# jakobblaabjerg/point-cloud-classifier

Measured on NVIDIA B200. Metric: train samples/sec (fwd+bwd), DeepSets B=256 N=1024, higher is better.
Workload: dtype bf16

## Files before the change

### point-cloud-classifier_b200/csrc/pcc_fused_bwd.cu

```cuda
#include "pcc_fused.cuh"
#include "pcc_head.cuh"

namespace pcc {

constexpr int kRingB = 3;

struct BwdParams {
  const float* x;
  const int64_t* offsets;
  int64_t n, B, num_tiles;
  int d, L, pooling, res_mask;
  const uint8_t* wpack;
  uint32_t w_off[kMaxLayers], wt_off[kMaxLayers];
  const float* bias[kMaxLayers];
  const float* dpooled;
  const int32_t* argmax;
  uint8_t* stage_h[kMaxLayers];
  uint8_t* stage_g[kMaxLayers];
  float* part_w[kMaxLayers];
  float* part_b[kMaxLayers];
  int virt;
  int nbig;
  const int32_t* row_set;
  const float* row_scale;
  long long* trace;
};

__device__ __forceinline__ void trace_b(long long* trace, int role, int& n, int id) {
  if (trace && blockIdx.x == 0 && n < 2047) {
    trace[role * 4096 + 2 * n] = id;
    trace[role * 4096 + 2 * n + 1] = clock64();
    ++n;
  }
}

struct BwdSmem {
  uint32_t bufG, bufH, ring, bias, bars, total;
};
__host__ __device__ inline BwdSmem bwd_smem(int H, int L) {
  BwdSmem s;
  uint32_t o = 0;
  s.bufG = o; o += kTileM * H * 2;
  s.bufH = o; o += kTileM * H * 2;
  s.ring = o; o += kRingB * w_slab_bytes(H);
  s.bias = o; o += (uint32_t)(L - 1) * H * 4;
  s.bars = o; o += 128;
  s.total = o;
  return s;
}

template <int H, int ACT>
__global__ void __launch_bounds__(kThreads, 1) phi_bwd_chain_kernel(const BwdParams p) {
  extern __shared__ __align__(1024) uint8_t smem[];
  const BwdSmem lay = bwd_smem(H, p.L);
  uint8_t* bufG = smem + lay.bufG;
  uint8_t* bufH = smem + lay.bufH;
  uint8_t* ring = smem + lay.ring;
  float* biasS = reinterpret_cast<float*>(smem + lay.bias);
  uint64_t* bars = reinterpret_cast<uint64_t*>(smem + lay.bars);
  uint64_t* full = bars;
  uint64_t* empty = bars + kRingB;
  uint64_t* a_ready = bars + 2 * kRingB;
  uint64_t* accA_ready = bars + 2 * kRingB + 1;
  uint64_t* accB_ready = bars + 2 * kRingB + 2;
  uint64_t* wf_ready = bars + 2 * kRingB + 3;
  uint32_t* tmem_slot = reinterpret_cast<uint32_t*>(bars + 2 * kRingB + 4);

  constexpr uint32_t SLAB = w_slab_bytes(H);
  constexpr uint32_t X_LBO = kTileM * 16;
  constexpr uint32_t W0_LBO = H * 16;
  constexpr uint32_t BLOB = kTileM * H * 2;
  constexpr int NSLAB = H / 64;
  constexpr int NCHUNK = H / 32;
  constexpr uint32_t ACC_A = 0, ACC_B = 256;

  const int warp = threadIdx.x >> 5, lane = threadIdx.x & 31;
  const int L = p.L;
  const int lh = L - 2;

  for (int i = threadIdx.x; i < (L - 1) * H; i += kThreads) biasS[i] = __ldg(p.bias[i / H] + (i % H));
  if (threadIdx.x == 0) {
    for (int i = 0; i < kRingB; ++i) { mbar_init(&full[i], 1); mbar_init(&empty[i], 1); }
    mbar_init(a_ready, kEpiWarps);
    mbar_init(accA_ready, 1);
    mbar_init(accB_ready, 1);
    mbar_init(wf_ready, 1);
    fence_mbar_init();
  }
  if (warp == kMmaWarp) tmem_alloc<512>(tmem_slot);
  tc_fence_before();
  __syncthreads();
  tc_fence_after();
  const uint32_t tmem = *tmem_slot;
  pdl_wait();
  const bool virt = p.virt != 0;
  const bool vmax = p.virt == 1, bcast = p.virt == 2;
  const bool bcast3 = bcast && p.L == 3;

  if (warp == kProdWarp) {
    if (lane == 0) {
      uint32_t stage = 0, phase = 0;
      auto push = [&](const uint8_t* src, uint32_t bytes) {
        mbar_wait(&empty[stage], phase ^ 1);
        mbar_arrive_expect_tx(&full[stage], bytes);
        bulk_g2s(ring + stage * SLAB, src, bytes, &full[stage]);
        if (++stage == kRingB) { stage = 0; phase ^= 1; }
      };
      auto push_layer = [&](uint32_t off) { for (int s = 0; s < NSLAB; ++s) push(p.wpack + off + (size_t)s * SLAB, SLAB); };
      for (int64_t tile = blockIdx.x; tile < p.num_tiles; tile += gridDim.x) {
        push(p.wpack + p.w_off[0], (kK0 / 8) * W0_LBO);
        if (!virt) push_layer(p.wt_off[L - 1]);
        if (L == 3) {
          push_layer(p.w_off[1]);
          push_layer(p.wt_off[1]);
          if (!bcast3) push(p.wpack + p.w_off[0], (kK0 / 8) * W0_LBO);
        }
      }
    }
  } else if (warp == kMmaWarp) {
    if (lane == 0) {
      constexpr uint32_t IDESC = make_idesc_bf16(128, H, 0, 0);
      uint32_t stage = 0, phase = 0, a_phase = 0;
      const uint32_t g_base = smem_u32(bufG), h_base = smem_u32(bufH), r_base = smem_u32(ring);
      auto wait_a = [&]() { mbar_wait(a_ready, a_phase); a_phase ^= 1; tc_fence_after(); };
      auto gemm = [&](uint32_t act_base, uint32_t acc_col, bool accumulate_first) {
        for (int s = 0; s < NSLAB; ++s) {
          mbar_wait(&full[stage], phase);
          tc_fence_after();
          const uint32_t w_slab = r_base + stage * SLAB;
#pragma unroll
          for (int ks = 0; ks < 4; ++ks)
            umma_bf16(tmem + acc_col, make_smem_desc_sw128_k(act_base + s * kActSlab + ks * 32),
                      make_smem_desc_sw128_k(w_slab + ks * 32), IDESC, ((s | ks) != 0) || accumulate_first);
          umma_commit(&empty[stage]);
          if (++stage == kRingB) { stage = 0; phase ^= 1; }
        }
      };
      auto gemm0 = [&]() {
        mbar_wait(&full[stage], phase);
        tc_fence_after();
        umma_bf16(tmem + ACC_A, make_smem_desc(h_base, X_LBO, 128), make_smem_desc(r_base + stage * SLAB, W0_LBO, 128),
                  IDESC, 0);
        umma_commit(&empty[stage]);
        if (++stage == kRingB) { stage = 0; phase ^= 1; }
      };
      for (int64_t tile = blockIdx.x; tile < p.num_tiles; tile += gridDim.x) {
        wait_a();
        gemm0();
        umma_commit(accA_ready);
        if (!virt) {
          wait_a();
          gemm(g_base, ACC_B, false);
          umma_commit(accB_ready);
        }
        if (L == 3) {
          wait_a();
          gemm(h_base, ACC_A, false);
          umma_commit(accA_ready);
          wait_a();
          gemm(bcast3 ? h_base : g_base, ACC_B, (p.res_mask >> 1) & 1);
          umma_commit(accB_ready);
          if (!bcast3) {
            wait_a();
            gemm0();
            umma_commit(accA_ready);
          }
        }
      }
    }
  } else {
    const int quarter = warp & 3, grp = warp >> 2;
    const int r = quarter * 32 + lane;
    const uint32_t lane_base = tmem + ((uint32_t)(quarter * 32) << 16);
    uint32_t phA = 0, phB = 0, wf_phase = 0;
    const int d = p.d;
    float xcur[kK0] = {}, xnext[kK0];
    auto load_x = [&](int64_t tile) {
      const int64_t row = tile * kTileM + r;
#pragma unroll
      for (int j = 0; j < kK0; ++j)
        xnext[j] = (grp == 0 && j < d && row < p.n && tile < p.num_tiles) ? __ldg(p.x + row * d + j) : 0.f;
    };
    auto stage_x = [&]() {
      if (grp == 0) {
        *reinterpret_cast<uint4*>(bufH + r * 16) = make_uint4(pack_bf16x2(xcur[0], xcur[1]), pack_bf16x2(xcur[2], xcur[3]),
                                                              pack_bf16x2(xcur[4], xcur[5]), pack_bf16x2(xcur[6], xcur[7]));
        *reinterpret_cast<uint4*>(bufH + X_LBO + r * 16) =
            make_uint4(pack_bf16x2(xcur[8], xcur[9]), pack_bf16x2(xcur[10], xcur[11]), pack_bf16x2(xcur[12], xcur[13]),
                       pack_bf16x2(xcur[14], xcur[15]));
      }
    };
    auto acquire = [&]() {
      if (threadIdx.x == 0) bulk_wait_read0();
      asm volatile("bar.sync 1, 256;" ::: "memory");
    };
    auto store_blob = [&](uint8_t* gdst, const uint8_t* sbuf) {
      fence_proxy_async();
      asm volatile("bar.sync 1, 256;" ::: "memory");
      if (threadIdx.x == 0) { bulk_s2g(gdst, sbuf, BLOB); bulk_commit(); }
    };
    auto store_slabs = [&](uint8_t* gdst, const uint8_t* sbuf, int s0, int count, uint8_t* gdst2, const uint8_t* sbuf2) {
      fence_proxy_async();
      asm volatile("bar.sync 1, 256;" ::: "memory");
      if (threadIdx.x == 0) {
        bulk_s2g(gdst + (size_t)s0 * kActSlab, sbuf + (size_t)s0 * kActSlab, (uint32_t)count * kActSlab);
        if (gdst2) bulk_s2g(gdst2 + (size_t)s0 * kActSlab, sbuf2 + (size_t)s0 * kActSlab, (uint32_t)count * kActSlab);
        bulk_commit();
      }
    };
    auto wait_A = [&]() { mbar_wait(accA_ready, phA); phA ^= 1; tc_fence_after(); };
    auto wait_B = [&]() { mbar_wait(accB_ready, phB); phB ^= 1; tc_fence_after(); };
    auto arrive_a = [&]() { tc_fence_before(); fence_proxy_async(); mbar_arrive_warp(a_ready); };
    auto h_chunk8 = [&](const uint32_t* z, const float* bl, uint8_t* dst, bool res) {
      const float4 b0 = *reinterpret_cast<const float4*>(bl);
      const float4 b1 = *reinterpret_cast<const float4*>(bl + 4);
      const uint64_t bb[4] = {f32x2(b0.x, b0.y), f32x2(b0.z, b0.w), f32x2(b1.x, b1.y), f32x2(b1.z, b1.w)};
      uint4 old = make_uint4(0u, 0u, 0u, 0u);
      if (res) old = *reinterpret_cast<const uint4*>(dst);
      const uint32_t oo[4] = {old.x, old.y, old.z, old.w};
      uint32_t pk[4];
#pragma unroll
      for (int j = 0; j < 4; ++j) {
        uint64_t o = act2<ACT>(fadd2(f32x2(__uint_as_float(z[2 * j]), __uint_as_float(z[2 * j + 1])), bb[j]));
        if (res) o = fadd2(o, bf16x2_to_f32x2(oo[j]));
        pk[j] = pack_bf16x2_pair(o);
      }
      *reinterpret_cast<uint4*>(dst) = make_uint4(pk[0], pk[1], pk[2], pk[3]);
    };
    auto hda_chunk8 = [&](const uint32_t* z, const float* bl, uint8_t* hdst, uint8_t* dadst) {
      const float4 b0 = *reinterpret_cast<const float4*>(bl);
      const float4 b1 = *reinterpret_cast<const float4*>(bl + 4);
      const uint64_t bb[4] = {f32x2(b0.x, b0.y), f32x2(b0.z, b0.w), f32x2(b1.x, b1.y), f32x2(b1.z, b1.w)};
      uint32_t ph[4], pd[4];
#pragma unroll
      for (int j = 0; j < 4; ++j) {
        uint64_t a, da;
        act_and_grad2<ACT>(fadd2(f32x2(__uint_as_float(z[2 * j]), __uint_as_float(z[2 * j + 1])), bb[j]), a, da);
        ph[j] = pack_bf16x2_pair(a);
        pd[j] = pack_bf16x2_pair(da);
      }
      *reinterpret_cast<uint4*>(hdst) = make_uint4(ph[0], ph[1], ph[2], ph[3]);
      *reinterpret_cast<uint4*>(dadst) = make_uint4(pd[0], pd[1], pd[2], pd[3]);
    };
    auto dz_chunk8 = [&](const uint32_t* z, const uint32_t* g, const float* bl, uint8_t* dst) {
      const float4 b0 = *reinterpret_cast<const float4*>(bl);
      const float4 b1 = *reinterpret_cast<const float4*>(bl + 4);
      const uint64_t bb[4] = {f32x2(b0.x, b0.y), f32x2(b0.z, b0.w), f32x2(b1.x, b1.y), f32x2(b1.z, b1.w)};
      uint32_t pk[4];
#pragma unroll
      for (int j = 0; j < 4; ++j) {
        uint64_t a, da;
        act_and_grad2<ACT>(fadd2(f32x2(__uint_as_float(z[2 * j]), __uint_as_float(z[2 * j + 1])), bb[j]), a, da);
        pk[j] = pack_bf16x2_pair(fmul2(f32x2(__uint_as_float(g[2 * j]), __uint_as_float(g[2 * j + 1])), da));
      }
      *reinterpret_cast<uint4*>(dst) = make_uint4(pk[0], pk[1], pk[2], pk[3]);
    };
    auto hdz_chunk8 = [&](const uint32_t* z, const uint32_t* g, const float* bl, uint8_t* hdst, uint8_t* gdst, bool res) {
      const float4 b0 = *reinterpret_cast<const float4*>(bl);
      const float4 b1 = *reinterpret_cast<const float4*>(bl + 4);
      const uint64_t bb[4] = {f32x2(b0.x, b0.y), f32x2(b0.z, b0.w), f32x2(b1.x, b1.y), f32x2(b1.z, b1.w)};
      uint4 old = make_uint4(0u, 0u, 0u, 0u);
      if (res) old = *reinterpret_cast<const uint4*>(hdst);
      const uint32_t oo[4] = {old.x, old.y, old.z, old.w};
      uint32_t ph[4], pg[4];
#pragma unroll
      for (int j = 0; j < 4; ++j) {
        uint64_t a, da;
        act_and_grad2<ACT>(fadd2(f32x2(__uint_as_float(z[2 * j]), __uint_as_float(z[2 * j + 1])), bb[j]), a, da);
        if (res) a = fadd2(a, bf16x2_to_f32x2(oo[j]));
        ph[j] = pack_bf16x2_pair(a);
        pg[j] = pack_bf16x2_pair(fmul2(f32x2(__uint_as_float(g[2 * j]), __uint_as_float(g[2 * j + 1])), da));
      }
      *reinterpret_cast<uint4*>(hdst) = make_uint4(ph[0], ph[1], ph[2], ph[3]);
      *reinterpret_cast<uint4*>(gdst) = make_uint4(pg[0], pg[1], pg[2], pg[3]);
    };

    load_x(blockIdx.x);
    int tn = 0;
    const bool tr0 = threadIdx.x == 0;
#define TRE(id) do { if (tr0) trace_b(p.trace, 0, tn, id); } while (0)
    for (int64_t tile = blockIdx.x; tile < p.num_tiles; tile += gridDim.x) {
      const int64_t r0 = tile * kTileM;
      const int64_t row = r0 + r;
#pragma unroll
      for (int j = 0; j < kK0; ++j) xcur[j] = xnext[j];
      TRE(0);
      stage_x();
      arrive_a();
      TRE(2);
      load_x(tile + gridDim.x);
      const int64_t myset = (!vmax && row < p.n) ? (int64_t)__ldg(p.row_set + row) : -1;
      const float scale = (!vmax && row < p.n) ? __ldg(p.row_scale + row) : 0.f;
      const float gs = vmax ? ((row < p.n) ? __ldg(p.dpooled + row) : 0.f) : 1.f;

      acquire();
      TRE(1);
      if (vmax) {
        if (threadIdx.x == 0) {
          const uint32_t f0 = (uint32_t)(r0 % H);
          mbar_arrive_expect_tx(wf_ready, NSLAB * kActSlab);
          for (int s = 0; s < NSLAB; ++s)
            bulk_g2s(bufG + s * kActSlab, p.wpack + p.w_off[L - 1] + (size_t)s * SLAB + (size_t)f0 * 128, kActSlab, wf_ready);
        }
      } else if (!bcast3) {
        float* gS = reinterpret_cast<float*>(bufH + 16384);
        int* aS = reinterpret_cast<int*>(bufH + 16384 + H * 4);
        const int64_t last_row = (r0 + kTileM - 1 < p.n - 1) ? r0 + kTileM - 1 : p.n - 1;
        const int64_t b_lo = __ldg(p.row_set + r0), b_hi = __ldg(p.row_set + last_row);
        const bool is_max = (p.pooling == PCC_POOL_MAX) && !bcast;
        if (myset < 0) {
          for (int kc = grp; kc < H / 8; kc += 2)
            *reinterpret_cast<uint4*>(bufG + act_chunk_off(r, kc * 8)) = make_uint4(0u, 0u, 0u, 0u);
        }
        for (int64_t b = (b_lo < 0 ? 0 : b_lo); b <= b_hi; ++b) {
          asm volatile("bar.sync 1, 256;" ::: "memory");
          for (int i = threadIdx.x; i < H; i += kEpiThreads) {
            gS[i] = __ldg(p.dpooled + b * H + i);
            if (is_max) aS[i] = __ldg(p.argmax + b * H + i);
          }
          asm volatile("bar.sync 1, 256;" ::: "memory");
          if (myset == b) {
            const int rr = (int)row;
#pragma unroll 2
            for (int kc = grp; kc < H / 8; kc += 2) {
              const float4 g0 = *reinterpret_cast<const float4*>(gS + kc * 8);
              const float4 g1 = *reinterpret_cast<const float4*>(gS + kc * 8 + 4);
              float o[8] = {g0.x, g0.y, g0.z, g0.w, g1.x, g1.y, g1.z, g1.w};
              if (is_max) {
                const int4 a0 = *reinterpret_cast<const int4*>(aS + kc * 8);
                const int4 a1 = *reinterpret_cast<const int4*>(aS + kc * 8 + 4);
                o[0] = a0.x == rr ? o[0] : 0.f; o[1] = a0.y == rr ? o[1] : 0.f; o[2] = a0.z == rr ? o[2] : 0.f;
                o[3] = a0.w == rr ? o[3] : 0.f; o[4] = a1.x == rr ? o[4] : 0.f; o[5] = a1.y == rr ? o[5] : 0.f;
                o[6] = a1.z == rr ? o[6] : 0.f; o[7] = a1.w == rr ? o[7] : 0.f;
              } else {
#pragma unroll
                for (int j = 0; j < 8; ++j) o[j] *= scale;
              }
              *reinterpret_cast<uint4*>(bufG + act_chunk_off(r, kc * 8)) =
                  make_uint4(pack_bf16x2(o[0], o[1]), pack_bf16x2(o[2], o[3]), pack_bf16x2(o[4], o[5]), pack_bf16x2(o[6], o[7]));
            }
          }
        }
      }
      TRE(3);
      if (!virt) {
        store_blob(p.stage_g[L - 1] + (size_t)tile * BLOB, bufG);
        arrive_a();
      }
      TRE(4);

      if (bcast3) {
        wait_A();
        TRE(5);
        const float* bl = biasS;
#pragma unroll 1
        for (int c = grp; c < NCHUNK; c += 2) {
          uint32_t z[32];
          tmem_ld32(lane_base + ACC_A + c * 32, z);
          tmem_wait_ld();
#pragma unroll
          for (int q = 0; q < 4; ++q) {
            const uint32_t off = act_chunk_off(r, c * 32 + q * 8);
            hda_chunk8(z + q * 8, bl + c * 32 + q * 8, bufH + off, bufG + off);
          }
          store_slabs(p.stage_h[0] + (size_t)tile * BLOB, bufH, c >> 1, 1, nullptr, nullptr);
        }
        TRE(6);
        arrive_a();
        TRE(7);
      } else if (L == 3) {
        wait_A();
        TRE(5);
        const float* bl = biasS;
        uint32_t va[32], vb[32];
        tmem_ld32(lane_base + ACC_A + grp * 32, va);
#pragma unroll 1
        for (int c = grp; c < NCHUNK; c += 4) {
          tmem_wait_ld();
          if (c + 2 < NCHUNK) tmem_ld32(lane_base + ACC_A + (c + 2) * 32, vb);
#pragma unroll
          for (int q = 0; q < 4; ++q) h_chunk8(va + q * 8, bl + c * 32 + q * 8, bufH + act_chunk_off(r, c * 32 + q * 8), false);
          if (c + 2 < NCHUNK) {
            tmem_wait_ld();
            if (c + 4 < NCHUNK) tmem_ld32(lane_base + ACC_A + (c + 4) * 32, va);
#pragma unroll
            for (int q = 0; q < 4; ++q)
              h_chunk8(vb + q * 8, bl + (c + 2) * 32 + q * 8, bufH + act_chunk_off(r, (c + 2) * 32 + q * 8), false);
          }
          store_slabs(p.stage_h[0] + (size_t)tile * BLOB, bufH, (c - grp) >> 1, (c + 2 < NCHUNK) ? 2 : 1, nullptr, nullptr);
        }
        TRE(6);
        arrive_a();
        TRE(7);
      }

      if (!virt) wait_B();
      TRE(8);
      wait_A();
      TRE(9);
      acquire();
      TRE(10);
      if (bcast3) {
        const bool res = (p.res_mask >> lh) & 1;
        const float* bl = biasS + lh * H;
        const float* grow = p.dpooled + (myset < 0 ? 0 : myset) * H;
        const float sc = myset < 0 ? 0.f : scale;
        uint32_t gn[32];
        auto load_g = [&](int c, uint32_t (&dst)[32]) {
#pragma unroll
          for (int j = 0; j < 8; ++j) {
            const float4 t4 = __ldg(reinterpret_cast<const float4*>(grow + c * 32) + j);
            dst[4 * j] = __float_as_uint(t4.x); dst[4 * j + 1] = __float_as_uint(t4.y);
            dst[4 * j + 2] = __float_as_uint(t4.z); dst[4 * j + 3] = __float_as_uint(t4.w);
          }
        };
        load_g(grp, gn);
#pragma unroll 1
        for (int c = grp; c < NCHUNK; c += 2) {
          uint32_t z[32], g[32];
          tmem_ld32(lane_base + ACC_A + c * 32, z);
#pragma unroll
          for (int j = 0; j < 32; ++j) g[j] = __float_as_uint(sc * __uint_as_float(gn[j]));
          if (c + 2 < NCHUNK) load_g(c + 2, gn);
          if (res) tmem_st32(lane_base + ACC_B + c * 32, g);
          tmem_wait_ld();
#pragma unroll
          for (int q = 0; q < 4; ++q)
            dz_chunk8(z + q * 8, g + q * 8, bl + c * 32 + q * 8, bufH + act_chunk_off(r, c * 32 + q * 8));
          store_slabs(p.stage_g[lh] + (size_t)tile * BLOB, bufH, c >> 1, 1, nullptr, nullptr);
        }
        if (res) tmem_wait_st();
      } else if (virt) {
        if (vmax) {
          mbar_wait(wf_ready, wf_phase);
          wf_phase ^= 1;
        }
        const bool res = (p.res_mask >> lh) & 1;
        const float* bl = biasS + lh * H;
#pragma unroll 1
        for (int c = grp; c < NCHUNK; c += 2) {
          uint32_t z[32], g[32];
          tmem_ld32(lane_base + ACC_A + c * 32, z);
#pragma unroll
          for (int q = 0; q < 4; ++q) {
            const uint4 wv = *reinterpret_cast<const uint4*>(bufG + act_chunk_off(r, c * 32 + q * 8));
            g[q * 8 + 0] = __float_as_uint(gs * bf16_lo(wv.x)); g[q * 8 + 1] = __float_as_uint(gs * bf16_hi(wv.x));
            g[q * 8 + 2] = __float_as_uint(gs * bf16_lo(wv.y)); g[q * 8 + 3] = __float_as_uint(gs * bf16_hi(wv.y));
            g[q * 8 + 4] = __float_as_uint(gs * bf16_lo(wv.z)); g[q * 8 + 5] = __float_as_uint(gs * bf16_hi(wv.z));
            g[q * 8 + 6] = __float_as_uint(gs * bf16_lo(wv.w)); g[q * 8 + 7] = __float_as_uint(gs * bf16_hi(wv.w));
          }
          if (res) tmem_st32(lane_base + ACC_B + c * 32, g);
          tmem_wait_ld();
#pragma unroll
          for (int q = 0; q < 4; ++q) {
            const uint32_t off = act_chunk_off(r, c * 32 + q * 8);
            if (bcast) dz_chunk8(z + q * 8, g + q * 8, bl + c * 32 + q * 8, bufG + off);
            else hdz_chunk8(z + q * 8, g + q * 8, bl + c * 32 + q * 8, bufH + off, bufG + off, res);
          }
          if (bcast) store_slabs(p.stage_g[lh] + (size_t)tile * BLOB, bufG, c >> 1, 1, nullptr, nullptr);
          else store_slabs(p.stage_h[lh] + (size_t)tile * BLOB, bufH, c >> 1, 1, p.stage_g[lh] + (size_t)tile * BLOB, bufG);
        }
        if (res) tmem_wait_st();
      } else {
        const bool res = (p.res_mask >> lh) & 1;
        const float* bl = biasS + lh * H;
#pragma unroll 1
        for (int c = grp; c < NCHUNK; c += 2) {
          uint32_t z[32], g[32];
          tmem_ld32(lane_base + ACC_A + c * 32, z);
          tmem_ld32(lane_base + ACC_B + c * 32, g);
          tmem_wait_ld();
#pragma unroll
          for (int q = 0; q < 4; ++q) {
            const uint32_t off = act_chunk_off(r, c * 32 + q * 8);
            hdz_chunk8(z + q * 8, g + q * 8, bl + c * 32 + q * 8, bufH + off, bufG + off, res);
          }
          store_slabs(p.stage_h[lh] + (size_t)tile * BLOB, bufH, c >> 1, 1, p.stage_g[lh] + (size_t)tile * BLOB, bufG);
        }
      }
      TRE(11);
      TRE(12);

      if (L == 3) {
        arrive_a();
        if (threadIdx.x == 0) bulk_wait_read0();
        asm volatile("bar.sync 1, 256;" ::: "memory");
        TRE(13);
        if (bcast3) {
          wait_B();
          TRE(14);
          TRE(15);
#pragma unroll 1
          for (int c = grp; c < NCHUNK; c += 2) {
            uint32_t g[32];
            tmem_ld32(lane_base + ACC_B + c * 32, g);
            tmem_wait_ld();
#pragma unroll
            for (int q = 0; q < 4; ++q) {
              uint8_t* dst = bufG + act_chunk_off(r, c * 32 + q * 8);
              const uint4 da = *reinterpret_cast<const uint4*>(dst);
              const uint32_t dd[4] = {da.x, da.y, da.z, da.w};
              uint32_t pk[4];
#pragma unroll
              for (int j = 0; j < 4; ++j)
                pk[j] = pack_bf16x2_pair(fmul2(f32x2(__uint_as_float(g[q * 8 + 2 * j]), __uint_as_float(g[q * 8 + 2 * j + 1])),
                                               bf16x2_to_f32x2(dd[j])));
              *reinterpret_cast<uint4*>(dst) = make_uint4(pk[0], pk[1], pk[2], pk[3]);
            }
            store_slabs(p.stage_g[0] + (size_t)tile * BLOB, bufG, c >> 1, 1, nullptr, nullptr);
          }
        } else {
        stage_x();
        arrive_a();
        wait_B();
        wait_A();
        TRE(14);
        acquire();
        TRE(15);
        const float* bl = biasS;
#pragma unroll 1
        for (int c = grp; c < NCHUNK; c += 2) {
          uint32_t z[32], g[32];
          tmem_ld32(lane_base + ACC_A + c * 32, z);
          tmem_ld32(lane_base + ACC_B + c * 32, g);
          tmem_wait_ld();
#pragma unroll
          for (int q = 0; q < 4; ++q)
            dz_chunk8(z + q * 8, g + q * 8, bl + c * 32 + q * 8, bufG + act_chunk_off(r, c * 32 + q * 8));
          store_slabs(p.stage_g[0] + (size_t)tile * BLOB, bufG, c >> 1, 1, nullptr, nullptr);
        }
        }
        TRE(16);
        TRE(17);
      }
    }
#undef TRE
    if (threadIdx.x == 0) bulk_wait0();
  }

  tc_fence_before();
  __syncthreads();
  if (warp == kMmaWarp) tmem_dealloc<512>(tmem);
}

constexpr int kSlots = 6;

struct WgradJob {
  int layer;
  int64_t first, stride;
  int slot;
};
__host__ __device__ inline int wgrad_members(int grid, int nbig, int layer) {
  if (layer == 0) return grid;
  return (grid - (layer - 1) + nbig - 1) / nbig;
}
__device__ inline WgradJob wgrad_job(int j, int cta, int grid, int nbig) {
  WgradJob w;
  if (j == 0) {
    w.layer = 1 + cta % nbig;
    w.first = cta / nbig;
    w.stride = wgrad_members(grid, nbig, w.layer);
    w.slot = cta / nbig;
  } else {
    w.layer = 0; w.first = cta; w.stride = grid; w.slot = cta;
  }
  return w;
}

__device__ __forceinline__ int64_t wgrad_last_tile(const WgradJob& jb, int64_t num_tiles) {
  if (jb.first >= num_tiles) return jb.first - jb.stride;
  return jb.first + (num_tiles - 1 - jb.first) / jb.stride * jb.stride;
}

template <int H>
__global__ void __launch_bounds__(kThreads, 1) phi_wgrad_kernel(const BwdParams p) {
  extern __shared__ __align__(1024) uint8_t smem[];
  constexpr uint32_t BLOB = kTileM * H * 2;
  constexpr uint32_t HBLOB = BLOB / 2;
  constexpr uint32_t HSLAB = kActSlab / 2;
  constexpr int NSL = H / 64;
  constexpr uint32_t XBLOB = kTileM * kK0 * 2;
  constexpr int HALVES = H / 128;
  constexpr int CH = H / 8;
  constexpr int CPW = CH / kEpiWarps;
  uint8_t* slots = smem;
  uint8_t* bufX = smem + kSlots * HBLOB;
  uint64_t* bars = reinterpret_cast<uint64_t*>(smem + kSlots * HBLOB + 2 * XBLOB);
  uint64_t* full = bars;
  uint64_t* empty = bars + kSlots;
  uint64_t* x_full = bars + 2 * kSlots;
  uint64_t* x_empty = bars + 2 * kSlots + 2;
  uint64_t* acc_ready = bars + 2 * kSlots + 4;
  uint64_t* acc_free = bars + 2 * kSlots + 5;
  uint32_t* tmem_slot = reinterpret_cast<uint32_t*>(bars + 2 * kSlots + 6);

  const int warp = threadIdx.x >> 5, lane = threadIdx.x & 31;
  const int j0 = (p.nbig == 0) ? 1 : 0;
  if (threadIdx.x == 0) {
    for (int i = 0; i < kSlots; ++i) { mbar_init(&full[i], 1); mbar_init(&empty[i], 1 + kEpiWarps); }
    for (int i = 0; i < 2; ++i) { mbar_init(&x_full[i], kEpiWarps); mbar_init(&x_empty[i], 1); }
    mbar_init(acc_ready, 1);
    mbar_init(acc_free, kEpiWarps);
    fence_mbar_init();
  }
  if (warp == kMmaWarp) tmem_alloc<512>(tmem_slot);
  tc_fence_before();
  __syncthreads();
  tc_fence_after();
  const uint32_t tmem = *tmem_slot;
  pdl_wait();

  if (warp == kProdWarp) {
    if (lane == 0) {
      uint32_t stage = 0, phase = 0;
      auto push = [&](const uint8_t* src, int hf) {
        mbar_wait(&empty[stage], phase ^ 1);
        mbar_arrive_expect_tx(&full[stage], HBLOB);
        for (int sl = 0; sl < NSL; ++sl)
          bulk_g2s(slots + stage * HBLOB + sl * HSLAB, src + (size_t)sl * kActSlab + (size_t)hf * HSLAB, HSLAB, &full[stage]);
        if (++stage == kSlots) { stage = 0; phase ^= 1; }
      };
      for (int j = 1; j >= j0; --j) {
        const WgradJob jb = wgrad_job(j, blockIdx.x, gridDim.x, p.nbig);
        const int l = jb.layer;
        for (int64_t tile = wgrad_last_tile(jb, p.num_tiles); tile >= jb.first; tile -= jb.stride) {
          for (int hf = 0; hf < 2; ++hf) {
            push(p.stage_g[l] + (size_t)tile * BLOB, hf);
            if (l >= 1) push(p.stage_h[l - 1] + (size_t)tile * BLOB, hf);
          }
        }
      }
    }
  } else if (warp == kMmaWarp) {
    if (lane == 0) {
      uint32_t stage = 0, phase = 0, xpar = 0, xphase = 0 , free_phase = 0;
      const uint32_t s_base = smem_u32(slots), x_base = smem_u32(bufX);
      for (int j = 1; j >= j0; --j) {
        const WgradJob jb = wgrad_job(j, blockIdx.x, gridDim.x, p.nbig);
        const int l = jb.layer;
        const int Np = (l == 0) ? kK0 : H;
        const uint32_t idesc = make_idesc_bf16(128, Np, 1, 1);
        if (j < 1) { mbar_wait(acc_free, free_phase); free_phase ^= 1; tc_fence_after(); }
        bool first = true;
        for (int64_t tile = wgrad_last_tile(jb, p.num_tiles); tile >= jb.first; tile -= jb.stride) {
          uint32_t x_addr = 0;
          if (l == 0) {
            mbar_wait(&x_full[xpar], (xphase >> xpar) & 1);
            xphase ^= 1u << xpar;
            x_addr = x_base + xpar * XBLOB;
          }
          for (int hf = 0; hf < 2; ++hf) {
            const uint32_t g_stage = stage;
            mbar_wait(&full[stage], phase);
            if (++stage == kSlots) { stage = 0; phase ^= 1; }
            uint32_t in_addr = 0, in_stage = 0;
            if (l >= 1) {
              in_stage = stage;
              mbar_wait(&full[stage], phase);
              if (++stage == kSlots) { stage = 0; phase ^= 1; }
              in_addr = s_base + in_stage * HBLOB;
            }
            tc_fence_after();
            const uint32_t g_addr = s_base + g_stage * HBLOB;
#pragma unroll
            for (int o = 0; o < HALVES; ++o)
              for (int ks = 0; ks < kTileM / 32; ++ks) {
                const uint64_t a_desc = make_smem_desc_sw128_mn(g_addr + o * (2 * HSLAB) + ks * 2048, HSLAB);
                const uint64_t b_desc = (l >= 1) ? make_smem_desc_sw128_mn(in_addr + ks * 2048, HSLAB)
                                                 : make_smem_desc(x_addr + (hf * (kTileM / 32) + ks) * 256, 128, kTileM * 16);
                umma_bf16(tmem + o * Np, a_desc, b_desc, idesc, !(first && hf == 0 && ks == 0));
              }
            umma_commit(&empty[g_stage]);
            if (l >= 1) umma_commit(&empty[in_stage]);
          }
          first = false;
          if (l == 0) { umma_commit(&x_empty[xpar]); xpar ^= 1; }
        }
        umma_commit(acc_ready);
      }
    }
  } else {
    const int quarter = warp & 3, grp = warp >> 2;
    const int r = quarter * 32 + lane;
    const uint32_t lane_base = tmem + ((uint32_t)(quarter * 32) << 16);
    uint32_t stage = 0, phase = 0, xpar = 0, xphase = 0, acc_phase = 0;
    const int d = p.d;
    for (int j = 1; j >= j0; --j) {
      const WgradJob jb = wgrad_job(j, blockIdx.x, gridDim.x, p.nbig);
      const int l = jb.layer;
      const int Np = (l == 0) ? kK0 : H;
      float dbacc[CPW][8];
#pragma unroll
      for (int i = 0; i < CPW; ++i)
#pragma unroll
        for (int j = 0; j < 8; ++j) dbacc[i][j] = 0.f;
      for (int64_t tile = wgrad_last_tile(jb, p.num_tiles); tile >= jb.first; tile -= jb.stride) {
        if (l == 0) {
          mbar_wait(&x_empty[xpar], ((xphase >> xpar) & 1) ^ 1);
          xphase ^= 1u << xpar;
          if (grp == 0) {
            const int64_t row = tile * kTileM + r;
            float xr[kK0];
#pragma unroll
            for (int j = 0; j < kK0; ++j) xr[j] = (j < d && row < p.n) ? __ldg(p.x + row * d + j) : 0.f;
            uint8_t* xb = bufX + xpar * XBLOB;
            *reinterpret_cast<uint4*>(xb + r * 16) = make_uint4(pack_bf16x2(xr[0], xr[1]), pack_bf16x2(xr[2], xr[3]),
                                                                pack_bf16x2(xr[4], xr[5]), pack_bf16x2(xr[6], xr[7]));
            *reinterpret_cast<uint4*>(xb + kTileM * 16 + r * 16) =
                make_uint4(pack_bf16x2(xr[8], xr[9]), pack_bf16x2(xr[10], xr[11]), pack_bf16x2(xr[12], xr[13]),
                           pack_bf16x2(xr[14], xr[15]));
          }
          fence_proxy_async();
          mbar_arrive_warp(&x_full[xpar]);
          xpar ^= 1;
        }
        for (int hf = 0; hf < 2; ++hf) {
          mbar_wait(&full[stage], phase);
          const uint8_t* gb = slots + stage * HBLOB;
#pragma unroll
          for (int i = 0; i < CPW; ++i) {
            const int c = warp + kEpiWarps * i;
#pragma unroll
            for (int rr = 0; rr < 2; ++rr) {
              const int rw = lane + 32 * rr;
              const uint4 u = *reinterpret_cast<const uint4*>(gb + (uint32_t)(c >> 3) * HSLAB + (uint32_t)rw * 128u +
                                                              ((uint32_t)((c & 7) ^ (rw & 7)) << 4));
              dbacc[i][0] += bf16_lo(u.x); dbacc[i][1] += bf16_hi(u.x); dbacc[i][2] += bf16_lo(u.y); dbacc[i][3] += bf16_hi(u.y);
              dbacc[i][4] += bf16_lo(u.z); dbacc[i][5] += bf16_hi(u.z); dbacc[i][6] += bf16_lo(u.w); dbacc[i][7] += bf16_hi(u.w);
            }
          }
          mbar_arrive_warp(&empty[stage]);
          if (++stage == kSlots) { stage = 0; phase ^= 1; }
          if (l >= 1) {
            mbar_wait(&full[stage], phase);
            mbar_arrive_warp(&empty[stage]);
            if (++stage == kSlots) { stage = 0; phase ^= 1; }
          }
        }
      }
      float* pb = p.part_b[l] + (size_t)jb.slot * H;
#pragma unroll
      for (int i = 0; i < CPW; ++i)
#pragma unroll
        for (int j = 0; j < 8; ++j) {
          float s = warp_sum(dbacc[i][j]);
          if (lane == 0) pb[(warp + kEpiWarps * i) * 8 + j] = s;
        }
      mbar_wait(acc_ready, acc_phase);
      acc_phase ^= 1;
      tc_fence_after();
      float* pw = p.part_w[l] + (size_t)jb.slot * H * Np;
      const int nchunk = (Np < 32) ? 1 : Np / 32;
      const int ncol = (Np < 32) ? Np : 32;
#pragma unroll 1
      for (int item = grp; item < HALVES * nchunk; item += 2) {
        const int o = item / nchunk, c = item % nchunk;
        uint32_t v[32];
        tmem_ld32(lane_base + o * Np + c * 32, v);
        tmem_wait_ld();
        float* dst = pw + (size_t)(c * 32) * H + (o * 128 + r);
        const bool has_tiles = jb.first < p.num_tiles;
#pragma unroll
        for (int q = 0; q < 32; ++q)
          if (q < ncol) dst[(size_t)q * H] = has_tiles ? __uint_as_float(v[q]) : 0.f;
      }
      tc_fence_before();
      mbar_arrive_warp(acc_free);
    }
  }
  tc_fence_before();
  __syncthreads();
  if (warp == kMmaWarp) tmem_dealloc<512>(tmem);
}

constexpr int kFwvThreads = 512;
template <int H>
__global__ void __launch_bounds__(kFwvThreads) final_wgrad_virtual_kernel(const uint8_t* __restrict__ stage_h,
                                                                  const float* __restrict__ dpooled, int64_t B,
                                                                  float* __restrict__ dw, float* __restrict__ db) {
  pdl_enter();
  constexpr int CH = H / 8, NG = kFwvThreads / CH;
  constexpr uint32_t BLOB = kTileM * H * 2;
  __shared__ float red[NG][CH][8];
  __shared__ float redb[NG];
  const int f = blockIdx.x;
  const int kc = threadIdx.x % CH, bg = threadIdx.x / CH;
  float acc[8];
#pragma unroll
  for (int j = 0; j < 8; ++j) acc[j] = 0.f;
  float gsum = 0.f;
  for (int64_t b0 = (B - 1) / (8 * NG) * (8 * NG) + bg; b0 >= 0; b0 -= 8 * NG) {
    float g[8];
    uint4 u[8];
#pragma unroll
    for (int i = 0; i < 8; ++i) {
      const int64_t b = b0 + (int64_t)i * NG;
      const int64_t row = (b < B ? b : 0) * H + f;
      g[i] = (b < B) ? __ldg(dpooled + row) : 0.f;
      u[i] = __ldg(reinterpret_cast<const uint4*>(stage_h + (size_t)(row / kTileM) * BLOB +
                                                  act_chunk_off((int)(row % kTileM), kc * 8)));
    }
#pragma unroll
    for (int i = 0; i < 8; ++i) {
      acc[0] = fmaf(g[i], bf16_lo(u[i].x), acc[0]); acc[1] = fmaf(g[i], bf16_hi(u[i].x), acc[1]);
      acc[2] = fmaf(g[i], bf16_lo(u[i].y), acc[2]); acc[3] = fmaf(g[i], bf16_hi(u[i].y), acc[3]);
      acc[4] = fmaf(g[i], bf16_lo(u[i].z), acc[4]); acc[5] = fmaf(g[i], bf16_hi(u[i].z), acc[5]);
      acc[6] = fmaf(g[i], bf16_lo(u[i].w), acc[6]); acc[7] = fmaf(g[i], bf16_hi(u[i].w), acc[7]);
      gsum += g[i];
    }
  }
#pragma unroll
  for (int j = 0; j < 8; ++j) red[bg][kc][j] = acc[j];
  if (kc == 0) redb[bg] = gsum;
  __syncthreads();
  if (threadIdx.x < H) {
    const int c = threadIdx.x >> 3, j = threadIdx.x & 7;
    float s = 0.f;
#pragma unroll
    for (int g = 0; g < NG; ++g) s += red[g][c][j];
    dw[(size_t)f * H + threadIdx.x] = s;
  }
  if (threadIdx.x == 0) {
    float s = 0.f;
#pragma unroll
    for (int g = 0; g < NG; ++g) s += redb[g];
    db[f] = s;
  }
}

struct ReduceParams {
  const float* part_w[kMaxLayers];
  const float* part_b[kMaxLayers];
  float* dw[kMaxLayers];
  float* db[kMaxLayers];
  int Kp[kMaxLayers], K[kMaxLayers], np[kMaxLayers];
  int vec_begin[kMaxLayers + 1];
  int L, H;
};
__global__ void __launch_bounds__(256) wgrad_reduce_kernel(const ReduceParams p) {
  pdl_enter();
  __shared__ float4 red[8][32];
  const int lane = threadIdx.x & 31, g = threadIdx.x >> 5;
  const int item = blockIdx.x * 32 + lane;
  int l = 0;
  while (l + 1 < p.L && item >= p.vec_begin[l + 1]) ++l;
  float4 s = make_float4(0.f, 0.f, 0.f, 0.f);
  const int local = item - p.vec_begin[l];
  const int vec_per_k = p.H / 4;
  const int k = local / vec_per_k, row4 = (local % vec_per_k) * 4;
  const bool valid = item < p.vec_begin[p.L];
  const bool is_bias = valid && (k == p.Kp[l]);
  if (valid) {
    const float* src = is_bias ? p.part_b[l] + row4 : p.part_w[l] + (size_t)k * p.H + row4;
    const size_t stride = is_bias ? (size_t)p.H : (size_t)p.H * p.Kp[l];
    for (int c = g; c < p.np[l]; c += 8) {
      const float4 t = __ldg(reinterpret_cast<const float4*>(src + c * stride));
      s.x += t.x; s.y += t.y; s.z += t.z; s.w += t.w;
    }
  }
  red[g][lane] = s;
  __syncthreads();
  if (g == 0 && valid) {
    float4 t = red[0][lane];
#pragma unroll
    for (int j = 1; j < 8; ++j) { t.x += red[j][lane].x; t.y += red[j][lane].y; t.z += red[j][lane].z; t.w += red[j][lane].w; }
    if (is_bias) {
      *reinterpret_cast<float4*>(p.db[l] + row4) = t;
    } else if (k < p.K[l]) {
      float* dst = p.dw[l] + (size_t)row4 * p.K[l] + k;
      dst[0] = t.x; dst[(size_t)p.K[l]] = t.y; dst[2 * (size_t)p.K[l]] = t.z; dst[3 * (size_t)p.K[l]] = t.w;
    }
  }
}

__global__ void zero_f32_kernel_b(float* p, int64_t n) {
  int64_t i = blockIdx.x * (int64_t)blockDim.x + threadIdx.x;
  if (i < n) p[i] = 0.f;
}

struct BwdWs {
  int64_t stage_h[kMaxLayers], stage_g[kMaxLayers], part_w[kMaxLayers], part_b[kMaxLayers];
  int64_t row_set, row_scale, gmat, bscale;
  int64_t total;
  int grid;
};
constexpr int kGridCap = 160;
static BwdWs bwd_ws(const pcc_phi_desc* d, int64_t n, int sms, int64_t B = 0) {
  BwdWs w{};
  const int H = d->hidden, L = d->n_layers;
  const int64_t tiles = cdiv(n, kTileM);
  if (sms > kGridCap) sms = kGridCap;
  w.grid = (int)(tiles < sms ? tiles : sms);
  if (w.grid < L - 1) w.grid = L - 1;
  if (w.grid < 1) w.grid = 1;
  int64_t o = 0;
  auto take = [&](int64_t bytes) { int64_t at = o; o = (o + bytes + 255) / 256 * 256; return at; };
  const int64_t blob = (int64_t)kTileM * H * 2;
  for (int l = 0; l <= L - 2; ++l) w.stage_h[l] = take(tiles * blob);
  for (int l = 0; l < L; ++l) w.stage_g[l] = take(tiles * blob);
  for (int l = 0; l < L; ++l) {
    w.part_w[l] = take((int64_t)kGridCap * H * ((l == 0) ? kK0 : H) * 4);
    w.part_b[l] = take((int64_t)kGridCap * H * 4);
  }
  w.row_set = take(n * 4);
  w.row_scale = take(n * 4);
  w.gmat = take(B * H * 4);
  w.bscale = take(B * 4);
  w.total = o;
  return w;
}

int64_t phi_bwd_workspace_bytes(const pcc_phi_desc* d, int64_t n, int64_t B) { return bwd_ws(d, n, kGridCap, B).total; }

__global__ void set_bscale_kernel(const int64_t* __restrict__ offsets, int64_t B, int pooling, float* __restrict__ bscale) {
  const int64_t b = blockIdx.x * (int64_t)blockDim.x + threadIdx.x;
  if (b >= B) return;
  const float n = (float)(offsets[b + 1] - offsets[b]);
  bscale[b] = (n <= 0.f) ? 0.f : (pooling == PCC_POOL_SUM ? sqrtf(n) : 1.f);
}

template <int H, int ACT>
static int launch_chain(const BwdParams& p, int grid, cudaStream_t st) {
  const BwdSmem lay = bwd_smem(H, p.L);
  auto kern = phi_bwd_chain_kernel<H, ACT>;
  cudaError_t e = cudaFuncSetAttribute(kern, cudaFuncAttributeMaxDynamicSharedMemorySize, (int)lay.total);
  if (e != cudaSuccess) return fail("pcc_deepsets_phi_pool_bwd", cudaGetErrorString(e));
  {
    ProfScope prof(1, st);
    launch_dep(kern, dim3(grid), dim3(kThreads), lay.total, st, p);
  }
  return 0;
}
template <int H>
static int launch_wgrad(const BwdParams& p, int grid, cudaStream_t st) {
  const int smem_bytes = kSlots * (kTileM * H * 2 / 2) + 2 * kTileM * kK0 * 2 + 256;
  auto kern = phi_wgrad_kernel<H>;
  cudaError_t e = cudaFuncSetAttribute(kern, cudaFuncAttributeMaxDynamicSharedMemorySize, smem_bytes);
  if (e != cudaSuccess) return fail("pcc_deepsets_phi_pool_bwd", cudaGetErrorString(e));
  {
    ProfScope prof(2, st);
    launch_dep(kern, dim3(grid), dim3(kThreads), smem_bytes, st, p);
  }
  return 0;
}

}

using namespace pcc;

extern "C" int pcc_deepsets_phi_pool_bwd(const pcc_phi_desc* d, const float* x, const int64_t* offsets, int64_t n,
                                         int64_t B, const float* dpooled, const int32_t* argmax, float* const* dw,
                                         float* const* db, void* ws, const void* wpack, int device, void* stream) {
  PCC_ENTER(device);
  if (check_phi_desc(d, __func__) != 0) return -1;
  cudaStream_t st = (cudaStream_t)stream;
  const int H = d->hidden, L = d->n_layers;
  const bool virt = d->pooling == PCC_POOL_MAX && argmax == nullptr;
  PCC_REQUIRE(!virt || n == B * H, "max pooling without argmax: x must hold the B*H gathered argmax rows");
  int sms = 148;
  cudaDeviceGetAttribute(&sms, cudaDevAttrMultiProcessorCount, device);
  const BwdWs wl = bwd_ws(d, n, sms, B);
  uint8_t* wsb = (uint8_t*)ws;
  const int64_t tiles = cdiv(n, kTileM);
  const bool bcast = d->pooling != PCC_POOL_MAX && argmax != nullptr;
  if (tiles == 0) {
    for (int l = 0; l < L; ++l) {
      const int64_t cnt = (int64_t)H * (l == 0 ? d->input_dim : H);
      PCC_K(zero_f32_kernel_b)<<<(unsigned)cdiv(cnt, 256), 256, 0, st>>>(dw[l], cnt);
      PCC_K(zero_f32_kernel_b)<<<(unsigned)cdiv(H, 256), 256, 0, st>>>(db[l], H);
    }
    return check_launch(__func__);
  }

  PCC_REQUIRE(wpack != nullptr, "packed weight images of the forward pass required");
  const PackLayout pl = pack_layout(L, H);

  BwdParams p{};
  p.x = x; p.offsets = offsets; p.n = n; p.B = B; p.num_tiles = tiles;
  p.d = d->input_dim; p.L = L; p.pooling = d->pooling; p.res_mask = d->residual_mask;
  p.wpack = (const uint8_t*)wpack; p.dpooled = dpooled; p.argmax = argmax;
  for (int l = 0; l < L; ++l) {
    p.w_off[l] = pl.w_off[l]; p.wt_off[l] = pl.wt_off[l]; p.bias[l] = d->b[l];
    p.stage_g[l] = wsb + wl.stage_g[l];
    if (l <= L - 2) p.stage_h[l] = wsb + wl.stage_h[l];
    p.part_w[l] = (float*)(wsb + wl.part_w[l]);
    p.part_b[l] = (float*)(wsb + wl.part_b[l]);
  }
  p.trace = (long long*)debug_trace_buffer();
  p.row_set = (const int32_t*)(wsb + wl.row_set);
  p.row_scale = (const float*)(wsb + wl.row_scale);
  p.virt = virt ? 1 : (bcast ? 2 : 0);
  p.nbig = (virt || bcast) ? L - 2 : L - 1;
  if (bcast) {
    float* bscale = (float*)(wsb + wl.bscale);
    float* G = (float*)(wsb + wl.gmat);
    const float* ph = reinterpret_cast<const float*>(argmax);
    PCC_K(set_bscale_kernel)<<<(unsigned)cdiv(B, 256), 256, 0, st>>>(offsets, B, d->pooling, bscale);
    HeadTileParams hp{};
    hp.act = PCC_ACT_RELU;
    HeadTileProb& pw = hp.prob[0];
    pw.A = HeadOperand{dpooled, nullptr, 1, H, 0, 0, 0};
    pw.B = HeadOperand{ph, nullptr, 1, H, 0, 0, 0};
    pw.I = H; pw.J = H; pw.KK = (int)B;
    pw.C = dw[L - 1]; pw.ldc = H; pw.colsum = db[L - 1]; pw.colsum_w = bscale;
    head_set_tiles(pw);
    HeadTileProb& pg = hp.prob[1];
    pg.A = HeadOperand{dpooled, nullptr, H, 1, 0, 0, 0};
    pg.B = HeadOperand{d->w[L - 1], nullptr, 1, H, 0, 0, 0};
    pg.I = (int)B; pg.J = H; pg.KK = H;
    pg.C = G; pg.ldc = H;
    head_set_tiles(pg);
    launch_head_tiles(hp, pw.tiles + pg.tiles, st);
    p.dpooled = G;
    p.argmax = nullptr;
  }
  if (!virt)
    PCC_K(seg_prep_kernel)<<<(unsigned)cdiv(n, 256), 256, 0, st>>>(offsets, n, B, tiles, d->pooling, nullptr,
                                                                  (int32_t*)(wsb + wl.row_set), (float*)(wsb + wl.row_scale));
  int rc = 0;
#define PCC_DISPATCH(HH)                                                                 \
  switch (d->act) {                                                                      \
    case PCC_ACT_RELU: rc = launch_chain<HH, PCC_ACT_RELU>(p, wl.grid, st); break;       \
    case PCC_ACT_GELU: rc = launch_chain<HH, PCC_ACT_GELU>(p, wl.grid, st); break;       \
    default: rc = launch_chain<HH, PCC_ACT_SILU>(p, wl.grid, st); break;                 \
  }
  if (H == 256) { PCC_DISPATCH(256) } else { PCC_DISPATCH(128) }
#undef PCC_DISPATCH
  if (rc != 0) return rc;
  if (virt) {
    auto fk = (H == 256) ? final_wgrad_virtual_kernel<256> : final_wgrad_virtual_kernel<128>;
    launch_dep(fk, dim3(H), dim3(kFwvThreads), 0, st, p.stage_h[L - 2], dpooled, B, dw[L - 1], db[L - 1]);
  }
  rc = (H == 256) ? launch_wgrad<256>(p, wl.grid, st) : launch_wgrad<128>(p, wl.grid, st);
  if (rc != 0) return rc;
  ReduceParams rp{};
  const int Lr = (virt || bcast) ? L - 1 : L;
  rp.L = Lr; rp.H = H;
  int items = 0;
  for (int l = 0; l < Lr; ++l) {
    rp.part_w[l] = p.part_w[l]; rp.part_b[l] = p.part_b[l]; rp.dw[l] = dw[l]; rp.db[l] = db[l];
    rp.K[l] = (l == 0) ? d->input_dim : H;
    rp.Kp[l] = (l == 0) ? kK0 : H;
    rp.np[l] = wgrad_members(wl.grid, p.nbig, l);
    rp.vec_begin[l] = items;
    items += (rp.Kp[l] + 1) * (H / 4);
  }
  rp.vec_begin[Lr] = items;
  launch_dep(wgrad_reduce_kernel, dim3((unsigned)cdiv(items, 32)), dim3(256), 0, st, rp);
  return check_launch(__func__);
}
```

Measured before the change: 1.164 million.

## Fuse layer-0 weight gradient into backward chain kernel for virtual-max L=3

Adds a templated L0 path to the backward chain kernel. For virtual max-pooling with three layers, it computes the layer-0 weight and bias gradient directly in TMEM with an extra UMMA per tile, appending a constant-one input column to produce the bias. Per-block partials are written straight out, so staging dz for layer 0 to global memory is no longer needed and the wgrad kernel skips that job. This trades the store plus reload of the layer-0 gradient blobs for extra MMA and epilogue work and a sync inside the chain kernel.

```diff
diff --git a/point-cloud-classifier_b200/csrc/pcc_fused_bwd.cu b/point-cloud-classifier_b200/csrc/pcc_fused_bwd.cu
--- a/point-cloud-classifier_b200/csrc/pcc_fused_bwd.cu
+++ b/point-cloud-classifier_b200/csrc/pcc_fused_bwd.cu
@@ -23,6 +23,7 @@
   int nbig;
   const int32_t* row_set;
   const float* row_scale;
+  int l0cc;
   long long* trace;
 };
 
@@ -49,7 +50,7 @@
   return s;
 }
 
-template <int H, int ACT>
+template <int H, int ACT, bool L0>
 __global__ void __launch_bounds__(kThreads, 1) phi_bwd_chain_kernel(const BwdParams p) {
   extern __shared__ __align__(1024) uint8_t smem[];
   const BwdSmem lay = bwd_smem(H, p.L);
@@ -75,7 +76,7 @@
   constexpr uint32_t ACC_A = 0, ACC_B = 256;
 
   const int warp = threadIdx.x >> 5, lane = threadIdx.x & 31;
-  const int L = p.L;
+  const int L = L0 ? 3 : p.L;
   const int lh = L - 2;
 
   for (int i = threadIdx.x; i < (L - 1) * H; i += kThreads) biasS[i] = __ldg(p.bias[i / H] + (i % H));
@@ -93,9 +94,9 @@
   tc_fence_after();
   const uint32_t tmem = *tmem_slot;
   pdl_wait();
-  const bool virt = p.virt != 0;
-  const bool vmax = p.virt == 1, bcast = p.virt == 2;
-  const bool bcast3 = bcast && p.L == 3;
+  const bool virt = L0 || p.virt != 0;
+  const bool vmax = L0 || p.virt == 1, bcast = !L0 && p.virt == 2;
+  const bool bcast3 = bcast && L == 3;
 
   if (warp == kProdWarp) {
     if (lane == 0) {
@@ -165,6 +166,17 @@
             gemm0();
             umma_commit(accA_ready);
           }
+          if (L0) {
+            constexpr uint32_t IDESC0 = make_idesc_bf16(128, kK0, 1, 1);
+            wait_a();
+#pragma unroll
+            for (int o = 0; o < H / 128; ++o)
+#pragma unroll
+              for (int ks = 0; ks < kTileM / 16; ++ks)
+                umma_bf16(tmem + ACC_A + o * kK0, make_smem_desc_sw128_mn(g_base + o * 2 * kActSlab + ks * 2048, kActSlab),
+                          make_smem_desc(h_base + ks * 256, 128, kTileM * 16), IDESC0, ks != 0);
+            umma_commit(accA_ready);
+          }
         }
       }
     }
@@ -180,7 +192,9 @@
 #pragma unroll
       for (int j = 0; j < kK0; ++j)
         xnext[j] = (grp == 0 && j < d && row < p.n && tile < p.num_tiles) ? __ldg(p.x + row * d + j) : 0.f;
+      if (L0) xnext[7] = 1.f;
     };
+    float dw0[8] = {};
     auto stage_x = [&]() {
       if (grp == 0) {
         *reinterpret_cast<uint4*>(bufH + r * 16) = make_uint4(pack_bf16x2(xcur[0], xcur[1]), pack_bf16x2(xcur[2], xcur[3]),
@@ -527,7 +541,18 @@
 #pragma unroll
           for (int q = 0; q < 4; ++q)
             dz_chunk8(z + q * 8, g + q * 8, bl + c * 32 + q * 8, bufG + act_chunk_off(r, c * 32 + q * 8));
-          store_slabs(p.stage_g[0] + (size_t)tile * BLOB, bufG, c >> 1, 1, nullptr, nullptr);
+          if (!L0) store_slabs(p.stage_g[0] + (size_t)tile * BLOB, bufG, c >> 1, 1, nullptr, nullptr);
+        }
+        if (L0) {
+          arrive_a();
+          wait_A();
+          if (grp < H / 128) {
+            uint32_t v[16];
+            tmem_ld16(lane_base + ACC_A + grp * kK0, v);
+            tmem_wait_ld();
+#pragma unroll
+            for (int k = 0; k < 8; ++k) dw0[k] += __uint_as_float(v[k]);
+          }
         }
         }
         TRE(16);
@@ -536,6 +561,11 @@
     }
 #undef TRE
     if (threadIdx.x == 0) bulk_wait0();
+    if (L0 && grp < H / 128) {
+      const int f = grp * 128 + r;
+      for (int k = 0; k < d; ++k) p.part_w[0][((size_t)blockIdx.x * d + k) * H + f] = dw0[k];
+      p.part_b[0][(size_t)blockIdx.x * H + f] = dw0[7];
+    }
   }
 
   tc_fence_before();
@@ -596,6 +626,7 @@
 
   const int warp = threadIdx.x >> 5, lane = threadIdx.x & 31;
   const int j0 = (p.nbig == 0) ? 1 : 0;
+  const int j1 = p.l0cc ? 0 : 1;
   if (threadIdx.x == 0) {
     for (int i = 0; i < kSlots; ++i) { mbar_init(&full[i], 1); mbar_init(&empty[i], 1 + kEpiWarps); }
     for (int i = 0; i < 2; ++i) { mbar_init(&x_full[i], kEpiWarps); mbar_init(&x_empty[i], 1); }
@@ -620,7 +651,7 @@
           bulk_g2s(slots + stage * HBLOB + sl * HSLAB, src + (size_t)sl * kActSlab + (size_t)hf * HSLAB, HSLAB, &full[stage]);
         if (++stage == kSlots) { stage = 0; phase ^= 1; }
       };
-      for (int j = 1; j >= j0; --j) {
+      for (int j = j1; j >= j0; --j) {
         const WgradJob jb = wgrad_job(j, blockIdx.x, gridDim.x, p.nbig);
         const int l = jb.layer;
         for (int64_t tile = wgrad_last_tile(jb, p.num_tiles); tile >= jb.first; tile -= jb.stride) {
@@ -635,12 +666,12 @@
     if (lane == 0) {
       uint32_t stage = 0, phase = 0, xpar = 0, xphase = 0 , free_phase = 0;
       const uint32_t s_base = smem_u32(slots), x_base = smem_u32(bufX);
-      for (int j = 1; j >= j0; --j) {
+      for (int j = j1; j >= j0; --j) {
         const WgradJob jb = wgrad_job(j, blockIdx.x, gridDim.x, p.nbig);
         const int l = jb.layer;
         const int Np = (l == 0) ? kK0 : H;
         const uint32_t idesc = make_idesc_bf16(128, Np, 1, 1);
-        if (j < 1) { mbar_wait(acc_free, free_phase); free_phase ^= 1; tc_fence_after(); }
+        if (j < j1) { mbar_wait(acc_free, free_phase); free_phase ^= 1; tc_fence_after(); }
         bool first = true;
         for (int64_t tile = wgrad_last_tile(jb, p.num_tiles); tile >= jb.first; tile -= jb.stride) {
           uint32_t x_addr = 0;
@@ -685,7 +716,7 @@
     const uint32_t lane_base = tmem + ((uint32_t)(quarter * 32) << 16);
     uint32_t stage = 0, phase = 0, xpar = 0, xphase = 0, acc_phase = 0;
     const int d = p.d;
-    for (int j = 1; j >= j0; --j) {
+    for (int j = j1; j >= j0; --j) {
       const WgradJob jb = wgrad_job(j, blockIdx.x, gridDim.x, p.nbig);
       const int l = jb.layer;
       const int Np = (l == 0) ? kK0 : H;
@@ -922,7 +953,7 @@
 template <int H, int ACT>
 static int launch_chain(const BwdParams& p, int grid, cudaStream_t st) {
   const BwdSmem lay = bwd_smem(H, p.L);
-  auto kern = phi_bwd_chain_kernel<H, ACT>;
+  auto kern = p.l0cc ? phi_bwd_chain_kernel<H, ACT, true> : phi_bwd_chain_kernel<H, ACT, false>;
   cudaError_t e = cudaFuncSetAttribute(kern, cudaFuncAttributeMaxDynamicSharedMemorySize, (int)lay.total);
   if (e != cudaSuccess) return fail("pcc_deepsets_phi_pool_bwd", cudaGetErrorString(e));
   {
@@ -991,6 +1022,7 @@
   p.row_scale = (const float*)(wsb + wl.row_scale);
   p.virt = virt ? 1 : (bcast ? 2 : 0);
   p.nbig = (virt || bcast) ? L - 2 : L - 1;
+  p.l0cc = (virt && L == 3) ? 1 : 0;
   if (bcast) {
     float* bscale = (float*)(wsb + wl.bscale);
     float* G = (float*)(wsb + wl.gmat);
@@ -1040,7 +1072,7 @@
   for (int l = 0; l < Lr; ++l) {
     rp.part_w[l] = p.part_w[l]; rp.part_b[l] = p.part_b[l]; rp.dw[l] = dw[l]; rp.db[l] = db[l];
     rp.K[l] = (l == 0) ? d->input_dim : H;
-    rp.Kp[l] = (l == 0) ? kK0 : H;
+    rp.Kp[l] = (l == 0) ? (p.l0cc ? d->input_dim : kK0) : H;
     rp.np[l] = wgrad_members(wl.grid, p.nbig, l);
     rp.vec_begin[l] = items;
     items += (rp.Kp[l] + 1) * (H / 4);
```

Measured after the change: 1.256 million (median of 6 runs). +7.9%, better.
